# Sistemas-Multimedia/VCF

Hardware: AMD Instinct MI355X
Metric: Mpixels/s encode (DCT+deadzone) at 4K (higher is better)
Workload: dtype f32; 1 GPU; dct_dz_encode 2160x3840x3 u8 RGB frames (4K), B=8, YCoCg, deadzone Q=32, subband layout, 64 frames/step/GPU resident in HBM; global_batch=64, block_size=8, QSS=32, parallelism=frame-sharded x1

## Files before the change

vcf_amd/csrc/ab/vcf_dct_dz_ab.hip:

```cpp
#include <hip/hip_runtime.h>

#include <algorithm>
#include <cstdint>

#include "vcf_amd.h"
#include "vcf_amd_ab.h"
#include "vcf_dct8.h"
#include "vcf_dct_block.h"
#include "vcf_internal.h"
#include "vcf_pipeline.h"

namespace vcf {
namespace {

typedef uint32_t u32x4 __attribute__((ext_vector_type(4)));
typedef uint32_t u32x2 __attribute__((ext_vector_type(2)));

constexpr int kTile = 256;
constexpr int kSegBytes = kTile * 3;
constexpr int kStageBytes = 64 * kSegBytes;

struct Geom {
    int H, W, Hp, Wp, top, left, nbx, nby, tiles_per_row;
    int nblocks, tiles_per_frame;
// ... 80 lines not shown
    constexpr int per_lane = nseg * cps / kTile;
    static_assert(nseg * cps % kTile == 0, "whole stores per lane");
    const int tid = threadIdx.x;
    u32x4 v[per_lane];
    uint32_t go[per_lane];
    bool edge[per_lane];
    const uint32_t segA = (uint32_t)g.nby * (uint32_t)g.Wp * 3u, segB = (uint32_t)g.nbx * 3u;
    if (FA && SUB && segA < (1u << 24)) {
        static_assert(!SUB || (cps == 48 && bpb == 3), "multiply-shift constants");
#pragma unroll
        for (int r = 0; r < per_lane; ++r) {
            const int q = tid + r * kTile;
            const int seg = (int)(__umul24((uint32_t)q, 21846u) >> 20);
            const int off = (q - seg * cps) << 4;
            const int blk = (int)(__umul24((uint32_t)off, 43691u) >> 17);
            go[r] = rowbase[blk] + __umul24((uint32_t)(seg >> 3), segA) + __umul24((uint32_t)(seg & 7), segB) +
                    (uint32_t)(off - blk * bpb);
            v[r] = *reinterpret_cast<const u32x4 *>(stage + seg * lds_stride + off);
            edge[r] = off < 128 || off + 16 > cps * 16 - 128;
        }
    } else {
#pragma unroll
        for (int r = 0; r < per_lane; ++r) {
            const int q = tid + r * kTile;
            const int seg = q / cps;
            const int off = (q - seg * cps) << 4;
            const int blk = off / bpb;
            go[r] = rowbase[blk] + seg_base<SUB>(g, seg) + (uint32_t)(off - blk * bpb);
            v[r] = *reinterpret_cast<const u32x4 *>(stage + seg * lds_stride + off);
            edge[r] = off < 128 || off + 16 > cps * 16 - 128;
        }
    }
#pragma unroll
    for (int r = 0; r < per_lane; ++r) {
        if (NT == 1 || (NT == 2 && !edge[r]))
            __builtin_nontemporal_store(v[r] ^ 0x80808080u, reinterpret_cast<u32x4 *>(frame + go[r]));
        else
            *reinterpret_cast<u32x4 *>(frame + go[r]) = v[r] ^ 0x80808080u;
    }
}

__device__ __forceinline__ void opaque(uint32_t (&raw)[8][6], uint32_t dep)
{
#pragma unroll
    for (int y = 0; y < 8; ++y)
#pragma unroll
        for (int w = 0; w < 6; ++w) asm volatile("" : "+v"(raw[y][w]) : "v"(dep));
}

template <bool PAD, int LD = 1, bool FA = false>
__device__ __forceinline__ void load_block(const Geom &g, const uint8_t *src, int by, int bx,
                                           uint32_t (&raw)[8][6])
{
    if (!PAD) {
        const uint8_t *blk = src + ((long long)by * 8 * g.W + bx * 8) * 3;
#pragma unroll
        for (int y = 0; y < 8; ++y) {
            const u32x2 *p = reinterpret_cast<const u32x2 *>(
                FA ? blk + (long long)y * (3LL * g.W) : src + ((long long)(by * 8 + y) * g.W + bx * 8) * 3);
            const u32x2 a = LD == 0 ? __builtin_nontemporal_load(p) : p[0];
            const u32x2 b = LD == 0 ? __builtin_nontemporal_load(p + 1) : p[1];
            const u32x2 c = LD == 0 ? __builtin_nontemporal_load(p + 2) : p[2];
            raw[y][0] = a.x; raw[y][1] = a.y; raw[y][2] = b.x;
            raw[y][3] = b.y; raw[y][4] = c.x; raw[y][5] = c.y;
        }
    } else {
#pragma unroll
        for (int y = 0; y < 8; ++y) {
            const int sy = by * 8 + y - g.top;
#pragma unroll
            for (int w = 0; w < 6; ++w) raw[y][w] = 0;
#pragma unroll
            for (int n = 0; n < 24; ++n) {
                const int sx = bx * 8 + n / 3 - g.left;
                uint32_t b = 0;
                if (sy >= 0 && sy < g.H && sx >= 0 && sx < g.W)
                    b = src[((long long)sy * g.W + sx) * 3 + n % 3];
                raw[y][n >> 2] |= b << ((n & 3) * 8);
            }
        }
    }
}

template <bool POW2, bool SUB, bool PERC, bool SDWA, bool PK = false, bool MEMONLY = false>
__device__ __forceinline__ void encode_block(uint32_t (&raw)[8][6], const EncConsts &K, const FinalK &rowk,
                                             uint8_t *stage, int tid)
{
    auto s0 = [&](int i, int j, uint32_t w) {
        if (SUB) stage[(i * 8 + j) * kSegBytes + tid * 3 + 0] = (uint8_t)w;
        else stage[i * (kTile * 24) + tid * 24 + j * 3 + 0] = (uint8_t)w;
    };
    auto s1 = [&](int i, int j, uint32_t w) {
        if (SUB) stage[(i * 8 + j) * kSegBytes + tid * 3 + 1] = (uint8_t)w;
        else stage[i * (kTile * 24) + tid * 24 + j * 3 + 1] = (uint8_t)w;
    };
    auto s2 = [&](int i, int j, uint32_t w) {
        if (SUB) stage[(i * 8 + j) * kSegBytes + tid * 3 + 2] = (uint8_t)w;
        else stage[i * (kTile * 24) + tid * 24 + j * 3 + 2] = (uint8_t)w;
    };
    if constexpr (MEMONLY) {
#pragma unroll
        for (int n = 0; n < 64; ++n) {
            const uint32_t w = raw[n >> 3][(n * 3 / 4) % 6] >> (8 * (n & 3));
            s0(n >> 3, n & 7, w);
            s1(n >> 3, n & 7, w >> 1);
            s2(n >> 3, n & 7, w >> 2);
        }
    } else if constexpr (PK && POW2 && !PERC) {
        encode_block_channel_pk<0>(raw, rowk, K.qd[0], s0);
        opaque(raw, (uint32_t)tid);
        encode_block_channel_pk<1>(raw, rowk, K.qd[0], s1);
        opaque(raw, (uint32_t)tid);
        encode_block_channel_pk<2>(raw, rowk, K.qd[0], s2);
    } else {
        encode_block_channel_fold<0, POW2, PERC, SDWA>(raw, rowk, K.qd, s0);
        opaque(raw, (uint32_t)tid);
        encode_block_channel_fold<1, POW2, PERC, SDWA>(raw, rowk, K.qd, s1);
        opaque(raw, (uint32_t)tid);
        encode_block_channel_fold<2, POW2, PERC, SDWA>(raw, rowk, K.qd, s2);
    }
}

template <bool POW2, bool SUB, bool PERC, bool PAD, bool SDWA = true, bool PK = false, bool MEMONLY = false,
          int STREAMS = 0, int NT = 0, bool XCD = true, int LD = 1, int PRIO = 15, bool FA = true>
__global__ __launch_bounds__(kTile) void dct_dz_encode_kernel(const uint8_t *__restrict__ rgb,
                                                              uint8_t *__restrict__ kout, Geom g,
                                                              EncConsts K, FinalK rowk)
{
    __shared__ __attribute__((aligned(16))) uint8_t stage[kStageBytes];
    __shared__ uint32_t rowbase[kTile];
    const int tid = threadIdx.x;
    long long frame = blockIdx.y;
    int tile = blockIdx.x;
    if (XCD) {
        const unsigned n = gridDim.x * gridDim.y, gid = blockIdx.y * gridDim.x + blockIdx.x;
        const unsigned q = n >> 3, r = n & 7, x = gid & 7;
        const unsigned t = x * q + min(x, r) + (gid >> 3);
        frame = t / gridDim.x;
        tile = (int)(t - (unsigned)frame * gridDim.x);
    }
    const int n0 = tile * kTile;
    const int nvalid = min(kTile, g.nblocks - n0);
    if (tid < nvalid) {
        int by, bx;
        tile_block(g, n0 + tid, by, bx);
        rowbase[tid] = block_rowbase<SUB>(g, by, bx);
        uint32_t raw[8][6];
        if (PRIO & 3) __builtin_amdgcn_s_setprio(PRIO & 3);
        load_block<PAD, LD, FA>(g, rgb + frame * g.in_stride, by, bx, raw);
        if (PRIO & 3) __builtin_amdgcn_s_setprio(0);
        encode_block<POW2, SUB, PERC, SDWA, PK, MEMONLY>(raw, K, rowk, stage, tid);
    }
    __syncthreads();
    if (PRIO >> 2) __builtin_amdgcn_s_setprio(PRIO >> 2);
    if (STREAMS) {
        const long long S = (long long)g.out_stride * gridDim.y / 64 / 4096 * 4096;
        const long long t = (long long)blockIdx.y * gridDim.x + blockIdx.x;
        const int shift = STREAMS == 2 ? 32 : 0;
        if (nvalid == kTile)
#pragma unroll
            for (int r = 0; r < 12; ++r) {
                const int q = tid + r * kTile, seg = q / 48, off = (q - seg * 48) * 16;
                if (t * 768 + shift + off + 16 <= S)
                    __builtin_nontemporal_store(*reinterpret_cast<const u32x4 *>(stage + q * 16),
                                                reinterpret_cast<u32x4 *>(kout + seg * S + t * 768 + shift + off));
            }
        return;
    }
    if (nvalid == kTile && g.vec) move_runs_full<SUB, NT, FA>(g, stage, rowbase, kout + frame * g.out_stride);
    else move_runs_tab<SUB, true>(g, stage, rowbase, kout + frame * g.out_stride, nvalid);
}

template <bool PK>
__global__ __launch_bounds__(kTile, 2) void dct_dz_encode_diag(uint8_t *__restrict__ kout, Geom g,
                                                               EncConsts K, FinalK rowk, long long nblocks)
{
    const long long gid = (long long)blockIdx.x * kTile + threadIdx.x;
    if (gid >= nblocks) return;
    uint32_t raw[8][6];
#pragma unroll
    for (int y = 0; y < 8; ++y)
#pragma unroll
        for (int w = 0; w < 6; ++w) raw[y][w] = (uint32_t)(gid * 2654435761u) ^ (y * 0x01010101u * (w + 1));
    uint32_t acc = 0;
    auto sink = [&](int i, int j, uint32_t w) { acc += w << ((i + j) & 7); };
    if constexpr (PK) {
        encode_block_channel_pk<0>(raw, rowk, K.qd[0], sink);
        opaque(raw, acc);
        encode_block_channel_pk<1>(raw, rowk, K.qd[0], sink);
        opaque(raw, acc);
        encode_block_channel_pk<2>(raw, rowk, K.qd[0], sink);
    } else {
        encode_block_channel_fold<0, true, false, true>(raw, rowk, K.qd, sink);
        opaque(raw, acc);
        encode_block_channel_fold<1, true, false, true>(raw, rowk, K.qd, sink);
        opaque(raw, acc);
        encode_block_channel_fold<2, true, false, true>(raw, rowk, K.qd, sink);
    }
    reinterpret_cast<uint32_t *>(kout)[gid] = acc;
}

__device__ __forceinline__ void wave_lds_fence()
{
    __builtin_amdgcn_fence(__ATOMIC_SEQ_CST, "wavefront");
    __builtin_amdgcn_wave_barrier();
}

template <int TB>
struct ColsSmem {
    float tr[TB][8][9];
    uint8_t stage[64 * TB * 3 + 8 * 32];
};

template <int TB, bool SUB>
__device__ __forceinline__ int cols_stage_off(int seg)
{
    return SUB ? seg * (TB * 3) + (seg >> 3) * 32 : seg * (TB * 24) + seg * 32;
}

template <int TB, bool POW2, bool SUB, bool PERC, bool PAD>
__global__ __launch_bounds__(TB * 8) void dct_dz_encode_cols(const uint8_t *__restrict__ rgb,
                                                              uint8_t *__restrict__ kout, Geom g,
                                                              EncConsts K, int tiles_per_row)
{
    __shared__ __attribute__((aligned(16))) ColsSmem<TB> sm;
    const int tid = threadIdx.x;
    const int lb = tid >> 3, x = tid & 7;
    const int by = blockIdx.x / tiles_per_row;
    const int bx0 = (blockIdx.x - by * tiles_per_row) * TB;
    const int nvalid = min(TB, g.nbx - bx0);
    const int bx = bx0 + lb;
    const uint8_t *src = rgb + blockIdx.y * g.in_stride;
    uint8_t *dst = kout + blockIdx.y * g.out_stride;
    if (lb < nvalid) {
// ... 445 lines not shown
}

void make_geom(int32_t H, int32_t W, Geom &g)
{
    g.H = H;
    g.W = W;
    g.Hp = (H + 7) / 8 * 8;
    g.Wp = (W + 7) / 8 * 8;
    g.top = (g.Hp - H) / 2;
    g.left = (g.Wp - W) / 2;
    g.nbx = g.Wp / 8;
    g.nby = g.Hp / 8;
    g.tiles_per_row = (g.nbx + kTile - 1) / kTile;
    g.nblocks = g.nbx * g.nby;
    g.tiles_per_frame = (g.nblocks + kTile - 1) / kTile;
    g.in_stride = (long long)H * W * 3;
    g.out_stride = (long long)g.Hp * g.Wp * 3;
    g.vec = (g.nbx % 16 == 0) ? 1 : 0;
}

int check_args(const void *a, const void *b, int64_t n_frames, int32_t H, int32_t W,
               int32_t block_size, int32_t Q, uint32_t flags, bool decode)
{
    if (!a || !b) return set_error(VCF_ERR_INVALID, "null buffer");
    if (n_frames < 0) return set_error(VCF_ERR_INVALID, "n_frames < 0");
    if (H <= 0 || W <= 0)
        return set_error(VCF_ERR_INVALID, "Input image must be a 3D array (height, width, channels).");
    if (block_size != 8)
        return set_error(VCF_ERR_INVALID, "block_size %d: the 8x8 kernels need B=8", block_size);
    if (Q < 1 || (decode && Q > 32767))
        return set_error(VCF_ERR_INVALID, "quantization step %d out of range", Q);
    if (!decode && (Q & (Q - 1)) != 0 && Q > (1 << 18))
        return set_error(VCF_ERR_UNSUPPORTED, "quantization step %d too large", Q);
    if (flags & ~(VCF_DCT_NO_SUBBANDS | VCF_DCT_PERCEPTUAL))
        return set_error(VCF_ERR_INVALID, "unknown flags 0x%x", flags);
    if ((long long)((H + 7) & ~7) * ((W + 7) & ~7) * 3 >= (1LL << 31))
        return set_error(VCF_ERR_INVALID, "frame too large");
    return VCF_OK;
}

}
}

using namespace vcf;

#define VCF_ENC_CASE(P2, SB, PC, PD)                                                      \
    if (pow2 == P2 && sub == SB && perc == PC && pad == PD)                               \
        hipLaunchKernelGGL((dct_dz_encode_kernel<P2, SB, PC, PD>), grid, dim3(kTile), 0,  \
                           (hipStream_t)stream, rgb_dev + f0 * g.in_stride,               \
                           k_dev + f0 * g.out_stride, g, K, rowk);

#define VCF_DEC_CASE(SB, PC, PD)                                                          \
    if (sub == SB && perc == PC && pad == PD)                                             \
        hipLaunchKernelGGL((dct_dz_decode_kernel<SB, PC, PD>), grid, dim3(kTile), 0,      \
                           (hipStream_t)stream, k_dev + f0 * g.out_stride,                \
                           rgb_dev + f0 * g.in_stride, g, (int)Q);

extern "C" {

int vcf_dct_padded_shape(int32_t H, int32_t W, int32_t block_size, int32_t *Hp, int32_t *Wp)
{
    if (!Hp || !Wp) return set_error(VCF_ERR_INVALID, "null pointer");
    if (H <= 0 || W <= 0 || block_size <= 0)
        return set_error(VCF_ERR_INVALID, "bad shape %d x %d / block %d", H, W, block_size);
    *Hp = (H + block_size - 1) / block_size * block_size;
    *Wp = (W + block_size - 1) / block_size * block_size;
    return VCF_OK;
}

int vcf_dct_dz_encode(const uint8_t *rgb_dev, int64_t n_frames, int32_t H, int32_t W,
                      int32_t block_size, int32_t Q, uint32_t flags, uint8_t *k_dev, void *stream)
{
    return vcf_dct_dz_encode_variant(0, rgb_dev, n_frames, H, W, block_size, Q, flags, k_dev, stream);
}

int vcf_dct_dz_encode_variant(int variant, const uint8_t *rgb_dev, int64_t n_frames, int32_t H,
                              int32_t W, int32_t block_size, int32_t Q, uint32_t flags,
                              uint8_t *k_dev, void *stream)
{
    if (block_size != 8 && variant == 0)
        return dct_any_encode_u8(rgb_dev, n_frames, H, W, block_size, Q, flags, k_dev, stream);
    int rc = check_args(rgb_dev, k_dev, n_frames, H, W, block_size, Q, flags, false);
    if (rc != VCF_OK) return rc;
    if (variant < 0 || variant > 19) return set_error(VCF_ERR_INVALID, "unknown encode variant %d", variant);
    if (n_frames == 0) return VCF_OK;
    Geom g;
    make_geom(H, W, g);
    if (variant == 18 || variant == 19) {
        const PipeShape ps{2, variant == 18 ? 2 : 4, false};
        return run_pipelined(n_frames, ps, (hipStream_t)stream,
                             [&](long long f0, long long n, hipStream_t cs, const PipeHook *) {
                                 return vcf_dct_dz_encode_variant(0, rgb_dev + f0 * g.in_stride, n, H, W, block_size,
                                                                  Q, flags, k_dev + f0 * g.out_stride, cs);
                             });
    }
    const bool pow2 = (Q & (Q - 1)) == 0;
    const bool sub = !(flags & VCF_DCT_NO_SUBBANDS);
    const bool perc = (flags & VCF_DCT_PERCEPTUAL) != 0;
    const bool pad = (g.Hp != H) || (g.Wp != W);
    EncConsts K;
    make_enc_consts(K, Q);
    const FinalK rowk = pow2 ? row_final_k(Q) : final_k(1.0f, 1.0f);
    if (variant == 2 || variant == 6) {
        if (!pow2) return set_error(VCF_ERR_INVALID, "diagnostic variant needs a power-of-two Q");
        const long long nblocks = (long long)n_frames * g.nbx * g.nby;
        if (variant == 6)
            hipLaunchKernelGGL(dct_dz_encode_diag<true>, dim3((unsigned)((nblocks + kTile - 1) / kTile)),
                               dim3(kTile), 0, (hipStream_t)stream, k_dev, g, K, rowk, nblocks);
        else
            hipLaunchKernelGGL(dct_dz_encode_diag<false>, dim3((unsigned)((nblocks + kTile - 1) / kTile)),
                               dim3(kTile), 0, (hipStream_t)stream, k_dev, g, K, rowk, nblocks);
        return hip_check(hipGetLastError(), "dct_dz_encode_diag launch");
    }
    if (variant == 4) {
        if (!(pow2 && sub && !perc && !pad)) return set_error(VCF_ERR_INVALID, "variant 4: pow2 Q, aligned, default flags");
        for (int64_t f0 = 0; f0 < n_frames; f0 += 65535) {
            const dim3 grid(g.tiles_per_frame, (unsigned)std::min<int64_t>(65535, n_frames - f0));
            hipLaunchKernelGGL((dct_dz_encode_kernel<true, true, false, false, false>), grid, dim3(kTile), 0,
                               (hipStream_t)stream, rgb_dev + f0 * g.in_stride, k_dev + f0 * g.out_stride, g, K, rowk);
        }
        return hip_check(hipGetLastError(), "variant 4 launch");
    }
    if (variant == 8 || variant == 9 || variant == 10) {
        if (!(sub && !pad)) return set_error(VCF_ERR_INVALID, "variant 8: aligned frames, subband layout");
        if (variant != 8 && n_frames > 65535) return set_error(VCF_ERR_INVALID, "variants 9/10: <= 65535 frames");
        for (int64_t f0 = 0; f0 < n_frames; f0 += 65535) {
            const dim3 grid(g.tiles_per_frame, (unsigned)std::min<int64_t>(65535, n_frames - f0));
            if (variant == 8)
                hipLaunchKernelGGL((dct_dz_encode_kernel<true, true, false, false, true, false, true>), grid,
                                   dim3(kTile), 0, (hipStream_t)stream, rgb_dev + f0 * g.in_stride,
                                   k_dev + f0 * g.out_stride, g, K, rowk);
            else if (variant == 9)
                hipLaunchKernelGGL((dct_dz_encode_kernel<true, true, false, false, true, false, true, 1>), grid,
                                   dim3(kTile), 0, (hipStream_t)stream, rgb_dev, k_dev, g, K, rowk);
            else
                hipLaunchKernelGGL((dct_dz_encode_kernel<true, true, false, false, true, false, true, 2>), grid,
                                   dim3(kTile), 0, (hipStream_t)stream, rgb_dev, k_dev, g, K, rowk);
        }
        return hip_check(hipGetLastError(), "variant 8 launch");
    }
    if (variant >= 12 && variant <= 16) {
        if (!(pow2 && !perc && sub && !pad)) return set_error(VCF_ERR_INVALID, "variants 12-16: pow2 Q, aligned, default flags");
        if (n_frames > 65535) return set_error(VCF_ERR_INVALID, "variants 12-16: <= 65535 frames");
        const dim3 grid(g.tiles_per_frame, (unsigned)n_frames);
#define VCF_ENC_PRIO(V, P) \
        if (variant == V) \
            hipLaunchKernelGGL((dct_dz_encode_kernel<true, true, false, false, true, true, false, 0, 0, true, 1, P>), grid, \
                               dim3(kTile), 0, (hipStream_t)stream, rgb_dev, k_dev, g, K, rowk);
        VCF_ENC_PRIO(12, 15) VCF_ENC_PRIO(13, 5) VCF_ENC_PRIO(14, 12) VCF_ENC_PRIO(15, 3) VCF_ENC_PRIO(16, 0)
#undef VCF_ENC_PRIO
        return hip_check(hipGetLastError(), "variant 12-16 launch");
    }
    if (variant == 17) {
        if (!(pow2 && !perc && sub && !pad)) return set_error(VCF_ERR_INVALID, "variant 17: pow2 Q, aligned, default flags");
        if (n_frames > 65535) return set_error(VCF_ERR_INVALID, "variant 17: <= 65535 frames");
        const dim3 grid(g.tiles_per_frame, (unsigned)n_frames);
        hipLaunchKernelGGL((dct_dz_encode_kernel<true, true, false, false, true, true, false, 0, 0, true, 1, 15, false>),
                           grid, dim3(kTile), 0, (hipStream_t)stream, rgb_dev, k_dev, g, K, rowk);
        return hip_check(hipGetLastError(), "variant 17 launch");
    }
    if (variant == 11) {
        if (!(pow2 && !perc && sub && !pad)) return set_error(VCF_ERR_INVALID, "variant 11: pow2 Q, aligned, default flags");
        if (n_frames > 65535) return set_error(VCF_ERR_INVALID, "variant 11: <= 65535 frames");
        const dim3 grid(g.tiles_per_frame, (unsigned)n_frames);
        hipLaunchKernelGGL((dct_dz_encode_kernel<true, true, false, false, true, true, false, 0, 0, true, 0>), grid,
                           dim3(kTile), 0, (hipStream_t)stream, rgb_dev, k_dev, g, K, rowk);
        return hip_check(hipGetLastError(), "variant 11 launch");
    }
    if (variant == 7 && pow2 && !perc && sub && !pad) {
        if (n_frames > 65535) return set_error(VCF_ERR_INVALID, "variant 7: <= 65535 frames");
        const dim3 grid(g.tiles_per_frame, (unsigned)n_frames);
        hipLaunchKernelGGL((dct_dz_encode_kernel<true, true, false, false, true, true, false, 0, 1, false>), grid,
                           dim3(kTile), 0, (hipStream_t)stream, rgb_dev, k_dev, g, K, rowk);
        return hip_check(hipGetLastError(), "variant 7 launch");
    }
    if ((variant == 5 || (variant == 0 && pow2 && !perc)) && pow2 && !perc) {
        for (int64_t f0 = 0; f0 < n_frames; f0 += 65535) {
            const dim3 grid(g.tiles_per_frame, (unsigned)std::min<int64_t>(65535, n_frames - f0));
#define VCF_ENC_PK(SB, PD)                                                                                  \
    if (sub == SB && pad == PD)                                                                             \
        hipLaunchKernelGGL((dct_dz_encode_kernel<true, SB, false, PD, true, true>), grid, dim3(kTile), 0,   \
                           (hipStream_t)stream, rgb_dev + f0 * g.in_stride, k_dev + f0 * g.out_stride, g, K, rowk);
            VCF_ENC_PK(true, false) else VCF_ENC_PK(true, true) else VCF_ENC_PK(false, false) else VCF_ENC_PK(false, true)
#undef VCF_ENC_PK
            rc = hip_check(hipGetLastError(), "dct_dz_encode_kernel (packed) launch");
            if (rc != VCF_OK) return rc;
        }
        return VCF_OK;
    }
    if (variant == 3) return launch_cols<128>(rgb_dev, n_frames, k_dev, g, K, pow2, sub, perc, pad, stream);
    for (int64_t f0 = 0; f0 < n_frames; f0 += 65535) {
        const dim3 grid(g.tiles_per_frame, (unsigned)std::min<int64_t>(65535, n_frames - f0));
        VCF_ENC_CASE(true, true, false, false) else VCF_ENC_CASE(true, true, false, true)
        else VCF_ENC_CASE(true, true, true, false) else VCF_ENC_CASE(true, true, true, true)
        else VCF_ENC_CASE(true, false, false, false) else VCF_ENC_CASE(true, false, false, true)
        else VCF_ENC_CASE(true, false, true, false) else VCF_ENC_CASE(true, false, true, true)
        else VCF_ENC_CASE(false, true, false, false) else VCF_ENC_CASE(false, true, false, true)
        else VCF_ENC_CASE(false, true, true, false) else VCF_ENC_CASE(false, true, true, true)
        else VCF_ENC_CASE(false, false, false, false) else VCF_ENC_CASE(false, false, false, true)
        else VCF_ENC_CASE(false, false, true, false) else VCF_ENC_CASE(false, false, true, true)
        rc = hip_check(hipGetLastError(), "dct_dz_encode_kernel launch");
        if (rc != VCF_OK) return rc;
    }
    return VCF_OK;
}

int vcf_dct_dz_decode(const uint8_t *k_dev, int64_t n_frames, int32_t H, int32_t W,
                      int32_t block_size, int32_t Q, uint32_t flags, uint8_t *rgb_dev, void *stream)
{
    return vcf_dct_dz_decode_variant(0, k_dev, n_frames, H, W, block_size, Q, flags, rgb_dev, stream);
}

int vcf_dct_dz_decode_variant(int variant, const uint8_t *k_dev, int64_t n_frames, int32_t H, int32_t W,
                              int32_t block_size, int32_t Q, uint32_t flags, uint8_t *rgb_dev, void *stream)
{
    if (block_size != 8 && variant == 0)
        return dct_any_decode_u8(k_dev, n_frames, H, W, block_size, Q, flags, rgb_dev, stream);
    int rc = check_args(k_dev, rgb_dev, n_frames, H, W, block_size, Q, flags, true);
    if (rc != VCF_OK) return rc;
    if (variant < 0 || variant > 13) return set_error(VCF_ERR_INVALID, "unknown decode variant %d", variant);
    if (n_frames == 0) return VCF_OK;
    Geom g;
    make_geom(H, W, g);
    const bool sub = !(flags & VCF_DCT_NO_SUBBANDS);
    const bool perc = (flags & VCF_DCT_PERCEPTUAL) != 0;
    const bool pad = (g.Hp != H) || (g.Wp != W);
    if (variant >= 3) {
        if (!(sub && !perc && !pad)) return set_error(VCF_ERR_INVALID, "decode variants 3/4: aligned, default flags");
        if (n_frames > 65535) return set_error(VCF_ERR_INVALID, "decode variants 3/4: <= 65535 frames");
        const int tpr = (g.nbx + 31) / 32;
        const dim3 grid(tpr * g.nby, (unsigned)n_frames);
        if (variant == 3)
            hipLaunchKernelGGL((dct_dz_decode_cols<32, true, false, false, true, true>), grid, dim3(256), 0,
                               (hipStream_t)stream, k_dev, rgb_dev, g, (int)Q, tpr);
        else if (variant == 4)
            hipLaunchKernelGGL((dct_dz_decode_cols<32, true, false, false, false, false>), grid, dim3(256), 0,
                               (hipStream_t)stream, k_dev, rgb_dev, g, (int)Q, tpr);
        else if (variant == 5)
            hipLaunchKernelGGL((dct_dz_decode_cols<32, true, false, false, false, true, 0>), grid, dim3(256), 0,
                               (hipStream_t)stream, k_dev, rgb_dev, g, (int)Q, tpr);
        else if (variant == 6)
            hipLaunchKernelGGL((dct_dz_decode_cols<32, true, false, false, false, true, 3, 1>), grid, dim3(256), 0,
// ... 40 lines not shown
```

vcf_amd/csrc/vcf_dct_block.h:

```cpp
#pragma once
#include <math.h>
#include <stdint.h>
#include <string.h>

#include "vcf_dct8.h"

#if defined(__HIP_DEVICE_COMPILE__)
#define VCF_OPAQUE(x) asm volatile("" : "+v"(x))
#define VCF_SCHED_FENCE() __builtin_amdgcn_sched_barrier(0)
#else
#define VCF_OPAQUE(x) ((void)0)
#define VCF_SCHED_FENCE() ((void)0)
#endif

#if defined(__HIPCC__)
#define VCF_HD_HOST __host__
#else
#define VCF_HD_HOST
#endif

namespace vcf {

constexpr unsigned char kYQ[64] = {
    16, 11, 10, 16, 24, 40, 51, 61,   12, 12, 14, 19, 26, 58, 60, 55,
// ... 449 lines not shown
template <int B1>
VCF_HD uint32_t twice_byte(uint32_t b)
{
#if defined(__HIP_DEVICE_COMPILE__) && VCF_SDWA_ASM
    constexpr int B0 = -1;
    const uint32_t a = 1;
    VCF_SDWA_FN("v_lshlrev_b32_sdwa")
#else
    return byte_sel<B1>(b) << 1;
#endif
}

template <int C, int X>
VCF_HD float ycocg_sdwa(const uint32_t (&row)[6], uint32_t magic)
{
    constexpr int nr = 3 * X, ng = 3 * X + 1, nb = 3 * X + 2;
    const uint32_t wr = row[nr >> 2], wg = row[ng >> 2], wb = row[nb >> 2];
    if (C == 0) {
        const uint32_t rb = add_sdwa<nr & 3, nb & 3>(wr, wb);
        return bits_as_float(rb + twice_byte<ng & 3>(wg) + magic) - (8388608.0f + 512.0f);
    }
    if (C == 1) {
        const uint32_t t = add_sdwa<-1, nr & 3>(magic, wr);
        return bits_as_float(sub_sdwa<-1, nb & 3>(t, wb)) - (8388608.0f + 256.0f);
    }
    const uint32_t rb = add_sdwa<nr & 3, nb & 3>(wr, wb);
    const uint32_t t = add_sdwa<-1, ng & 3>(magic - rb, wg);
    return bits_as_float(add_sdwa<-1, ng & 3>(t, wg)) - (8388608.0f + 512.0f);
}

template <int C>
VCF_HD constexpr uint32_t ycocg_magic_word()
{
    return C == 0 ? kMagicI : C == 1 ? kMagicI + 256u : kMagicI + 512u;
}

template <int C, int X, bool SDWA>
VCF_HD void fold_columns(const uint32_t (&raw)[8][6], uint32_t magic, const FinalK &colk, float (&v)[8][8],
                         float &dep)
{
    if constexpr (X < 8) {
        float col[8];
#pragma unroll
        for (int y = 0; y < 8; ++y)
            col[y] = SDWA ? ycocg_sdwa<C, X>(raw[y], magic)
                          : ycocg_magic<C>(byte_of(raw[y], 3 * X), byte_of(raw[y], 3 * X + 1),
                                           byte_of(raw[y], 3 * X + 2));
        chain8(col, dep);
        dct2_8f(col, colk);
#pragma unroll
        for (int y = 0; y < 8; ++y) v[y][X] = col[y];
        dep = col[0];
        fold_columns<C, X + 1, SDWA>(raw, magic, colk, v, dep);
    }
}

template <int C, bool POW2, bool PERC, bool SDWA = false, typename Sink>
VCF_HD void encode_block_channel_fold(const uint32_t (&raw)[8][6], const FinalK &rowk, const float (&qd)[4],
                                      Sink &&sink)
{
    constexpr float cs = C == 1 ? 0.5f : 0.25f;
    constexpr FinalK colk = POW2 ? final_k(cs * 0.25f, cs * 0.5f) : final_k(1.0f, 1.0f);
    float v[8][8];
    float dep = qd[0];
    uint32_t magic = ycocg_magic_word<C>();
    VCF_OPAQUE(magic);
    fold_columns<C, 0, SDWA>(raw, magic, colk, v, dep);
#pragma unroll
    for (int i = 0; i < 8; ++i) {
        chain8(v[i], dep);
        if (POW2) dct2_8f(v[i], rowk);
        else dct2_8r(v[i]);
        dep = v[i][0];
#pragma unroll
        for (int j = 0; j < 8; ++j) {
            float t = v[i][j];
            if (PERC) t = (float)((double)t * pweight<C>(i * 8 + j));
            const float q = POW2 ? t : quant_div<false>(t, qd[qexp<C>(i, j) - 3]);
            sink(i, j, (uint32_t)cvt_trunc_i32(q));
        }
    }
}

#if defined(__HIPCC__)
typedef float vcf_f2 __attribute__((ext_vector_type(2)));
typedef uint32_t vcf_u2 __attribute__((ext_vector_type(2)));

template <int C, int X>
VCF_HD uint32_t ycocg_bits_sdwa(const uint32_t (&row)[6], uint32_t magic)
{
    constexpr int nr = 3 * X, ng = 3 * X + 1, nb = 3 * X + 2;
    const uint32_t wr = row[nr >> 2], wg = row[ng >> 2], wb = row[nb >> 2];
    if (C == 0) return add_sdwa<nr & 3, nb & 3>(wr, wb) + twice_byte<ng & 3>(wg) + magic;
    if (C == 1) return sub_sdwa<-1, nb & 3>(add_sdwa<-1, nr & 3>(magic, wr), wb);
    const uint32_t rb = add_sdwa<nr & 3, nb & 3>(wr, wb);
    return add_sdwa<-1, ng & 3>(add_sdwa<-1, ng & 3>(magic - rb, wg), wg);
}

template <int C, int XP>
VCF_HD void fold_columns_pk(const uint32_t (&raw)[8][6], uint32_t magic, const FinalK &colk,
                            vcf_f2 (&v)[8][4], vcf_f2 &dep)
{
    if constexpr (XP < 4) {
        constexpr float centre = C == 1 ? 8388608.0f + 256.0f : 8388608.0f + 512.0f;
        vcf_f2 col[8];
#pragma unroll
        for (int y = 0; y < 8; ++y) {
            const vcf_u2 b = {ycocg_bits_sdwa<C, 2 * XP>(raw[y], magic),
                              ycocg_bits_sdwa<C, 2 * XP + 1>(raw[y], magic)};
            col[y] = __builtin_bit_cast(vcf_f2, b) - centre;
        }
        chain8(col, dep);
        dct2_8f(col, colk);
#pragma unroll
        for (int y = 0; y < 8; ++y) v[y][XP] = col[y];
        dep = col[0];
        fold_columns_pk<C, XP + 1>(raw, magic, colk, v, dep);
    }
}

template <int C, typename Sink>
VCF_HD void encode_block_channel_pk(const uint32_t (&raw)[8][6], const FinalK &rowk, float dep0, Sink &&sink)
{
    constexpr float cs = C == 1 ? 0.5f : 0.25f;
    constexpr FinalK colk = final_k(cs * 0.25f, cs * 0.5f);
    vcf_f2 v[8][4];
    vcf_f2 dep = {dep0, dep0};
    uint32_t magic = ycocg_magic_word<C>();
    VCF_OPAQUE(magic);
    fold_columns_pk<C, 0>(raw, magic, colk, v, dep);
#pragma unroll
    for (int p = 0; p < 4; ++p) {
        vcf_f2 r[8];
#pragma unroll
        for (int xp = 0; xp < 4; ++xp) {
            r[2 * xp] = __builtin_shufflevector(v[2 * p][xp], v[2 * p + 1][xp], 0, 2);
            r[2 * xp + 1] = __builtin_shufflevector(v[2 * p][xp], v[2 * p + 1][xp], 1, 3);
        }
        chain8(r, dep);
        dct2_8f(r, rowk);
        dep = r[0];
#pragma unroll
        for (int j = 0; j < 8; ++j) {
            sink(2 * p, j, (uint32_t)cvt_trunc_i32(r[j].x));
            sink(2 * p + 1, j, (uint32_t)cvt_trunc_i32(r[j].y));
        }
    }
}
#endif

VCF_HD uint32_t byte_at(const uint32_t (&K)[16], int n)
{
    return (K[n >> 2] >> (8 * (n & 3))) & 0xffu;
}

template <int C, bool PERC>
VCF_HD void decode_block_channel(const uint8_t (&kb)[64], int Q, uint32_t (&res)[32])
{
    double v[8][8];
#pragma unroll
    for (int n = 0; n < 64; ++n) {
        int16_t y = (int16_t)(Q * ((int)kb[n] - 128));
        if (PERC) {
            const float f = (float)((double)(float)y / pweight<C>(n));
            y = (int16_t)(int)f;
        }
        v[n >> 3][n & 7] = (double)y;
    }
#pragma unroll
    for (int x = 0; x < 8; ++x) {
        double col[8];
#pragma unroll
        for (int y = 0; y < 8; ++y) col[y] = v[y][x];
        dct3_8r(col);
#pragma unroll
        for (int y = 0; y < 8; ++y) v[y][x] = col[y];
    }
#pragma unroll
    for (int y = 0; y < 8; ++y) dct3_8r(v[y]);
#pragma unroll
    for (int n = 0; n < 32; ++n) {
        const uint32_t lo = (uint16_t)(int16_t)(int)(v[(2 * n) >> 3][(2 * n) & 7] * 0.0625);
        const uint32_t hi = (uint16_t)(int16_t)(int)(v[(2 * n + 1) >> 3][(2 * n + 1) & 7] * 0.0625);
        res[n] = lo | (hi << 16);
    }
#pragma unroll
    for (int n = 0; n < 32; ++n) VCF_OPAQUE(res[n]);
}

VCF_HD uint32_t clip_u8(int v)
{
    v = (int16_t)(v + 128);
    return (uint32_t)(v < 0 ? 0 : (v > 255 ? 255 : v));
}

VCF_HD int sample_of(const uint32_t (&p)[32], int n)
{
    return (int16_t)(uint16_t)(p[n >> 1] >> ((n & 1) * 16));
}

VCF_HD void to_rgb_row(const uint32_t (&Yv)[32], const uint32_t (&Co)[32], const uint32_t (&Cg)[32],
                       int y, uint32_t (&px)[24])
{
#pragma unroll
    for (int x = 0; x < 8; ++x) {
        const int n = y * 8 + x;
        const int yv = sample_of(Yv, n), co = sample_of(Co, n), cg = sample_of(Cg, n);
        px[3 * x + 0] = clip_u8((int16_t)(yv + co - cg));
        px[3 * x + 1] = clip_u8((int16_t)(yv + cg));
        px[3 * x + 2] = clip_u8((int16_t)(yv - co - cg));
    }
#pragma unroll
    for (int q = 0; q < 24; ++q) VCF_OPAQUE(px[q]);
}

// ... 2 lines not shown
```

vcf_amd/csrc/vcf_dct_dz.hip:

```cpp
#include <hip/hip_runtime.h>

#include <algorithm>
#include <cstdint>

#include "vcf_amd.h"
#include "vcf_dct8.h"
#include "vcf_dct_block.h"
#include "vcf_internal.h"

namespace vcf {
namespace {

typedef uint32_t u32x4 __attribute__((ext_vector_type(4)));
typedef uint32_t u32x2 __attribute__((ext_vector_type(2)));

constexpr int kTile = 256;

struct Geom {
    int H, W, Hp, Wp, top, left, nbx, nby, tiles_per_row;
    int nblocks, tiles_per_frame;
    long long in_stride, out_stride;
    int vec;
};

// ... 87 lines not shown
    if (SUB && segA < (1u << 24)) {
        static_assert(!SUB || bpb == 3, "multiply-shift constants");
#pragma unroll
        for (int r = 0; r < per_lane; ++r) {
            const int q = tid + r * T;
            const int seg = (int)(__umul24((uint32_t)q, DivCps<T>::m) >> DivCps<T>::s);
            const int off = (q - seg * cps) << 4;
            const int blk = (int)(__umul24((uint32_t)off, 683u) >> 11);
            go[r] = rowbase[blk] + __umul24((uint32_t)(seg >> 3), segA) + __umul24((uint32_t)(seg & 7), segB) +
                    (uint32_t)(off - blk * bpb);
            v[r] = *reinterpret_cast<const u32x4 *>(stage + seg * lds_stride + off);
        }
    } else {
#pragma unroll
        for (int r = 0; r < per_lane; ++r) {
            const int q = tid + r * T;
            const int seg = q / cps;
            const int off = (q - seg * cps) << 4;
            const int blk = off / bpb;
            go[r] = rowbase[blk] + seg_base<SUB>(g, seg) + (uint32_t)(off - blk * bpb);
            v[r] = *reinterpret_cast<const u32x4 *>(stage + seg * lds_stride + off);
        }
    }
#pragma unroll
    for (int r = 0; r < per_lane; ++r) *reinterpret_cast<u32x4 *>(frame + go[r]) = v[r] ^ 0x80808080u;
}

__device__ __forceinline__ void opaque(uint32_t (&raw)[8][6], uint32_t dep)
{
#pragma unroll
    for (int y = 0; y < 8; ++y)
#pragma unroll
        for (int w = 0; w < 6; ++w) asm volatile("" : "+v"(raw[y][w]) : "v"(dep));
}

template <bool PAD>
__device__ __forceinline__ void load_block(const Geom &g, const uint8_t *src, int by, int bx,
                                           uint32_t (&raw)[8][6])
{
    if (!PAD) {
        const uint8_t *blk = src + ((long long)by * 8 * g.W + bx * 8) * 3;
#pragma unroll
        for (int y = 0; y < 8; ++y) {
            const u32x2 *p = reinterpret_cast<const u32x2 *>(blk + (long long)y * (3LL * g.W));
            const u32x2 a = p[0], b = p[1], c = p[2];
            raw[y][0] = a.x; raw[y][1] = a.y; raw[y][2] = b.x;
            raw[y][3] = b.y; raw[y][4] = c.x; raw[y][5] = c.y;
        }
    } else {
#pragma unroll
        for (int y = 0; y < 8; ++y) {
            const int sy = by * 8 + y - g.top;
#pragma unroll
            for (int w = 0; w < 6; ++w) raw[y][w] = 0;
#pragma unroll
            for (int n = 0; n < 24; ++n) {
                const int sx = bx * 8 + n / 3 - g.left;
                uint32_t b = 0;
                if (sy >= 0 && sy < g.H && sx >= 0 && sx < g.W)
                    b = src[((long long)sy * g.W + sx) * 3 + n % 3];
                raw[y][n >> 2] |= b << ((n & 3) * 8);
            }
        }
    }
}

template <bool POW2, bool SUB, bool PERC, bool PK, int T = kTile>
__device__ __forceinline__ void encode_block(uint32_t (&raw)[8][6], const EncConsts &K, const FinalK &rowk,
                                             uint8_t *stage, int tid)
{
    auto s0 = [&](int i, int j, uint32_t w) {
        if (SUB) stage[(i * 8 + j) * (T * 3) + tid * 3 + 0] = (uint8_t)w;
        else stage[i * (T * 24) + tid * 24 + j * 3 + 0] = (uint8_t)w;
    };
    auto s1 = [&](int i, int j, uint32_t w) {
        if (SUB) stage[(i * 8 + j) * (T * 3) + tid * 3 + 1] = (uint8_t)w;
        else stage[i * (T * 24) + tid * 24 + j * 3 + 1] = (uint8_t)w;
    };
    auto s2 = [&](int i, int j, uint32_t w) {
        if (SUB) stage[(i * 8 + j) * (T * 3) + tid * 3 + 2] = (uint8_t)w;
        else stage[i * (T * 24) + tid * 24 + j * 3 + 2] = (uint8_t)w;
    };
    if constexpr (PK && POW2 && !PERC) {
        encode_block_channel_pk<0>(raw, rowk, K.qd[0], s0);
        opaque(raw, (uint32_t)tid);
        encode_block_channel_pk<1>(raw, rowk, K.qd[0], s1);
        opaque(raw, (uint32_t)tid);
        encode_block_channel_pk<2>(raw, rowk, K.qd[0], s2);
    } else {
        encode_block_channel_fold<0, POW2, PERC, true>(raw, rowk, K.qd, s0);
        opaque(raw, (uint32_t)tid);
        encode_block_channel_fold<1, POW2, PERC, true>(raw, rowk, K.qd, s1);
        opaque(raw, (uint32_t)tid);
        encode_block_channel_fold<2, POW2, PERC, true>(raw, rowk, K.qd, s2);
    }
}

template <bool POW2, bool SUB, bool PERC, bool PAD, bool PK, int T = kTile>
__global__ __launch_bounds__(T) void dct_dz_encode_kernel(const uint8_t *__restrict__ rgb,
                                                          uint8_t *__restrict__ kout, Geom g,
                                                          EncConsts K, FinalK rowk)
{
    __shared__ __attribute__((aligned(16))) uint8_t stage[64 * T * 3];
    __shared__ uint32_t rowbase[T];
    const int tid = threadIdx.x;
    const unsigned n = gridDim.x * gridDim.y, gid = blockIdx.y * gridDim.x + blockIdx.x;
    const unsigned q = n >> 3, r = n & 7, xcd = gid & 7;
    const unsigned t = xcd * q + min(xcd, r) + (gid >> 3);
    const long long frame = t / gridDim.x;
    const int tile = (int)(t - (unsigned)frame * gridDim.x);
    const int n0 = tile * T;
    const int nvalid = min(T, g.nblocks - n0);
    if (tid < nvalid) {
        int by, bx;
        tile_block(g, n0 + tid, by, bx);
        rowbase[tid] = block_rowbase<SUB>(g, by, bx);
        uint32_t raw[8][6];
        __builtin_amdgcn_s_setprio(3);
        load_block<PAD>(g, rgb + frame * g.in_stride, by, bx, raw);
        __builtin_amdgcn_s_setprio(0);
        encode_block<POW2, SUB, PERC, PK, T>(raw, K, rowk, stage, tid);
    }
    __syncthreads();
    __builtin_amdgcn_s_setprio(3);
    if (nvalid == T && g.vec) move_runs_full<SUB, T>(g, stage, rowbase, kout + frame * g.out_stride);
    else move_runs_tab<SUB, true, T>(g, stage, rowbase, kout + frame * g.out_stride, nvalid);
}

__device__ __forceinline__ void wave_lds_fence()
{
    __builtin_amdgcn_fence(__ATOMIC_SEQ_CST, "wavefront");
    __builtin_amdgcn_wave_barrier();
}

template <int TB, bool SUB>
__device__ __forceinline__ int cols_stage_off(int seg)
{
    return SUB ? seg * (TB * 3) + (seg >> 3) * 32 : seg * (TB * 24) + seg * 32;
}

template <int TB>
struct DecColsSmem {
    double tr[TB][8][9];
    double lut[256];
    uint8_t stage[64 * TB * 3 + 8 * 32];
};

template <int TB, bool SUB, bool PERC, bool PAD>
__global__ __launch_bounds__(TB * 8) void dct_dz_decode_cols(const uint8_t *__restrict__ kin,
                                                              uint8_t *__restrict__ rgb, Geom g, int Q,
                                                              int tiles_per_row)
{
    constexpr bool NTL = false, NTS = true;
    constexpr int PRIO = 3, DQ = 1, EPI = 1;
    __shared__ __attribute__((aligned(16))) DecColsSmem<TB> sm;
    const int tid = threadIdx.x;
    const int lb = tid >> 3, x = tid & 7;
    const int by = blockIdx.x / tiles_per_row;
    const int bx0 = (blockIdx.x - by * tiles_per_row) * TB;
    const int nvalid = min(TB, g.nbx - bx0);
    const int bx = bx0 + lb;
    const uint8_t *src = kin + blockIdx.y * g.out_stride;
    uint8_t *dst = rgb + blockIdx.y * g.in_stride;

    constexpr int nseg = SUB ? 64 : 8;
    auto seg_off = [&](int seg) -> uint32_t {
        return (uint32_t)(SUB ? seg_offset_sub(g, by, bx0, seg) : seg_offset_nosub(g, by, bx0, seg));
    };
    if (PRIO) __builtin_amdgcn_s_setprio(PRIO);
    const uint32_t runA = (uint32_t)g.nby * (uint32_t)g.Wp * 3u, runB = (uint32_t)g.nbx * 3u;
    const bool fast24 = EPI == 1 && SUB && runA < (1u << 24) && runB * 8u < (1u << 24);
    const uint32_t runBase = ((uint32_t)by * (uint32_t)g.Wp + (uint32_t)bx0) * 3u;
    if (g.vec && nvalid == TB && (TB * 3) % 16 == 0) {
        constexpr int cps = (SUB ? 3 * TB : 24 * TB) / 16, total = nseg * cps;
        constexpr uint32_t kDivM = ((1u << 18) + cps - 1) / cps;
        static_assert(total < 4096, "multiply-shift division range");
#pragma unroll
        for (int q0 = 0; q0 < total; q0 += TB * 8) {
            const int q = q0 + tid;
            if (total % (TB * 8) == 0 || q < total) {
                int seg, off;
                uint32_t so;
                if (fast24) {
                    seg = (int)(__umul24((uint32_t)q, kDivM) >> 18);
                    off = (q - seg * cps) << 4;
                    so = __umul24((uint32_t)(seg >> 3), runA) + __umul24((uint32_t)(seg & 7), runB) + runBase;
                } else {
                    seg = q / cps;
                    off = (q - seg * cps) << 4;
                    so = seg_off(seg);
                }
                const u32x4 *gp = reinterpret_cast<const u32x4 *>(src + so + off);
                *reinterpret_cast<u32x4 *>(sm.stage + cols_stage_off<TB, SUB>(seg) + off) =
                    NTL ? __builtin_nontemporal_load(gp) : *gp;
            }
        }
    } else {
        const int seg_len = SUB ? 3 * nvalid : 24 * nvalid, total = nseg * seg_len;
#pragma clang loop unroll(disable) vectorize(disable) interleave(disable)
        for (int q = tid; q < total; q += TB * 8) {
            const int seg = q / seg_len, off = q - seg * seg_len;
            sm.stage[cols_stage_off<TB, SUB>(seg) + off] = src[seg_off(seg) + off];
        }
    }
    if (PRIO) __builtin_amdgcn_s_setprio(0);
// ... 280 lines not shown
```

Measured before the change: 723,700 Mpixels/s.

## Skip row DCT for row pairs that quantize to zero across the wave

Before each row-pair DCT pass in the packed encode path, the code sums the absolute column-pass outputs. If a ballot shows every lane's pair falls below the deadzone threshold, the row transform and quantization are skipped. In the production kernel (SKIP=2) the zero bytes are no longer written per skipped row; the staging rows 2..7 are pre-cleared with vectorized LDS stores, so skipped rows read as zero and computed rows overwrite them. The cost is the extra abs-sum and ballot per row pair plus the bulk zero fill, which pays off only when high-frequency rows are zero across whole waves. Correctness rests on the conservative bound constant.

Result: faster. 873,700 Mpixels/s, median of 6 (+20.7%).

```diff
diff --git a/vcf_amd/csrc/ab/vcf_dct_dz_ab.hip b/vcf_amd/csrc/ab/vcf_dct_dz_ab.hip
--- a/vcf_amd/csrc/ab/vcf_dct_dz_ab.hip
+++ b/vcf_amd/csrc/ab/vcf_dct_dz_ab.hip
@@ -186,7 +186,7 @@
     }
 }
 
-template <bool POW2, bool SUB, bool PERC, bool SDWA, bool PK = false, bool MEMONLY = false>
+template <bool POW2, bool SUB, bool PERC, bool SDWA, bool PK = false, bool MEMONLY = false, int SKIP = 0>
 __device__ __forceinline__ void encode_block(uint32_t (&raw)[8][6], const EncConsts &K, const FinalK &rowk,
                                              uint8_t *stage, int tid)
 {
@@ -211,11 +211,11 @@
             s2(n >> 3, n & 7, w >> 2);
         }
     } else if constexpr (PK && POW2 && !PERC) {
-        encode_block_channel_pk<0>(raw, rowk, K.qd[0], s0);
+        encode_block_channel_pk<0, SKIP>(raw, rowk, K.qd[0], s0);
         opaque(raw, (uint32_t)tid);
-        encode_block_channel_pk<1>(raw, rowk, K.qd[0], s1);
+        encode_block_channel_pk<1, SKIP>(raw, rowk, K.qd[0], s1);
         opaque(raw, (uint32_t)tid);
-        encode_block_channel_pk<2>(raw, rowk, K.qd[0], s2);
+        encode_block_channel_pk<2, SKIP>(raw, rowk, K.qd[0], s2);
     } else {
         encode_block_channel_fold<0, POW2, PERC, SDWA>(raw, rowk, K.qd, s0);
         opaque(raw, (uint32_t)tid);
@@ -226,7 +226,7 @@
 }
 
 template <bool POW2, bool SUB, bool PERC, bool PAD, bool SDWA = true, bool PK = false, bool MEMONLY = false,
-          int STREAMS = 0, int NT = 0, bool XCD = true, int LD = 1, int PRIO = 15, bool FA = true>
+          int STREAMS = 0, int NT = 0, bool XCD = true, int LD = 1, int PRIO = 15, bool FA = true, int SKIP = 0>
 __global__ __launch_bounds__(kTile) void dct_dz_encode_kernel(const uint8_t *__restrict__ rgb,
                                                               uint8_t *__restrict__ kout, Geom g,
                                                               EncConsts K, FinalK rowk)
@@ -253,7 +253,7 @@
         if (PRIO & 3) __builtin_amdgcn_s_setprio(PRIO & 3);
         load_block<PAD, LD, FA>(g, rgb + frame * g.in_stride, by, bx, raw);
         if (PRIO & 3) __builtin_amdgcn_s_setprio(0);
-        encode_block<POW2, SUB, PERC, SDWA, PK, MEMONLY>(raw, K, rowk, stage, tid);
+        encode_block<POW2, SUB, PERC, SDWA, PK, MEMONLY, SKIP>(raw, K, rowk, stage, tid);
     }
     __syncthreads();
     if (PRIO >> 2) __builtin_amdgcn_s_setprio(PRIO >> 2);
@@ -865,7 +865,7 @@
         return dct_any_encode_u8(rgb_dev, n_frames, H, W, block_size, Q, flags, k_dev, stream);
     int rc = check_args(rgb_dev, k_dev, n_frames, H, W, block_size, Q, flags, false);
     if (rc != VCF_OK) return rc;
-    if (variant < 0 || variant > 19) return set_error(VCF_ERR_INVALID, "unknown encode variant %d", variant);
+    if (variant < 0 || variant > 21) return set_error(VCF_ERR_INVALID, "unknown encode variant %d", variant);
     if (n_frames == 0) return VCF_OK;
     Geom g;
     make_geom(H, W, g);
@@ -941,6 +941,24 @@
         hipLaunchKernelGGL((dct_dz_encode_kernel<true, true, false, false, true, true, false, 0, 0, true, 1, 15, false>),
                            grid, dim3(kTile), 0, (hipStream_t)stream, rgb_dev, k_dev, g, K, rowk);
         return hip_check(hipGetLastError(), "variant 17 launch");
+    }
+    if (variant == 20 || variant == 21) {
+        if (!(pow2 && !perc)) return set_error(VCF_ERR_INVALID, "variants 20/21: pow2 Q, no -p");
+        for (int64_t f0 = 0; f0 < n_frames; f0 += 65535) {
+            const dim3 grid(g.tiles_per_frame, (unsigned)std::min<int64_t>(65535, n_frames - f0));
+#define VCF_ENC_SKIP(SB, PD, SK)                                                                                   \
+    if (sub == SB && pad == PD && (variant == 21) == (SK == 1))                                                     \
+        hipLaunchKernelGGL((dct_dz_encode_kernel<true, SB, false, PD, true, true, false, 0, 0, true, 1, 15, true, SK>), \
+                           grid, dim3(kTile), 0, (hipStream_t)stream, rgb_dev + f0 * g.in_stride,                   \
+                           k_dev + f0 * g.out_stride, g, K, rowk);
+            VCF_ENC_SKIP(true, false, 0) else VCF_ENC_SKIP(true, true, 0) else VCF_ENC_SKIP(false, false, 0)
+            else VCF_ENC_SKIP(false, true, 0) else VCF_ENC_SKIP(true, false, 1) else VCF_ENC_SKIP(true, true, 1)
+            else VCF_ENC_SKIP(false, false, 1) else VCF_ENC_SKIP(false, true, 1)
+#undef VCF_ENC_SKIP
+            rc = hip_check(hipGetLastError(), "variant 20/21 launch");
+            if (rc != VCF_OK) return rc;
+        }
+        return VCF_OK;
     }
     if (variant == 11) {
         if (!(pow2 && !perc && sub && !pad)) return set_error(VCF_ERR_INVALID, "variant 11: pow2 Q, aligned, default flags");
diff --git a/vcf_amd/csrc/vcf_dct_block.h b/vcf_amd/csrc/vcf_dct_block.h
--- a/vcf_amd/csrc/vcf_dct_block.h
+++ b/vcf_amd/csrc/vcf_dct_block.h
@@ -555,6 +555,50 @@
     }
 }
 
+constexpr float kRowSkipC = 4.0f + 0.00390625f;
+
+VCF_HD float row_skip_scale(float qd0)
+{
+    return qd0 * kRowSkipC;
+}
+
+VCF_HD float abs_f(float x)
+{
+#if defined(__HIPCC__)
+    return __builtin_fabsf(x);
+#else
+    return fabsf(x);
+#endif
+}
+
+VCF_HD float abs_add(float a, float b)
+{
+    float s = abs_f(a) + abs_f(b);
+#if defined(__HIP_DEVICE_COMPILE__)
+    asm("" : "+v"(s));
+#endif
+    return s;
+}
+
+VCF_HD float row_abs_sum(float a0, float a1, float a2, float a3, float a4, float a5, float a6, float a7)
+{
+    return abs_add(abs_add(abs_add(a0, a1), abs_add(a2, a3)), abs_add(abs_add(a4, a5), abs_add(a6, a7)));
+}
+
+VCF_HD bool row_pair_is_zero(float sa, float sb, float kb)
+{
+    return __builtin_fmaxf(sa, sb) * kb < 1.0f;
+}
+
+VCF_HD bool wave_all(bool pred)
+{
+#if defined(__HIP_DEVICE_COMPILE__)
+    return __builtin_amdgcn_ballot_w64(!pred) == 0;
+#else
+    return pred;
+#endif
+}
+
 #if defined(__HIPCC__)
 typedef float vcf_f2 __attribute__((ext_vector_type(2)));
 typedef uint32_t vcf_u2 __attribute__((ext_vector_type(2)));
@@ -592,7 +636,7 @@
     }
 }
 
-template <int C, typename Sink>
+template <int C, int SKIP = 0, typename Sink>
 VCF_HD void encode_block_channel_pk(const uint32_t (&raw)[8][6], const FinalK &rowk, float dep0, Sink &&sink)
 {
     constexpr float cs = C == 1 ? 0.5f : 0.25f;
@@ -602,8 +646,24 @@
     uint32_t magic = ycocg_magic_word<C>();
     VCF_OPAQUE(magic);
     fold_columns_pk<C, 0>(raw, magic, colk, v, dep);
+    const float kb = row_skip_scale(dep0);
 #pragma unroll
     for (int p = 0; p < 4; ++p) {
+        if (SKIP && p > 0) {
+            const vcf_f2(&a)[4] = v[2 * p], (&b)[4] = v[2 * p + 1];
+            const float sa = row_abs_sum(a[0].x, a[0].y, a[1].x, a[1].y, a[2].x, a[2].y, a[3].x, a[3].y);
+            const float sb = row_abs_sum(b[0].x, b[0].y, b[1].x, b[1].y, b[2].x, b[2].y, b[3].x, b[3].y);
+            if (wave_all(row_pair_is_zero(sa, sb, kb))) {
+                if (SKIP == 1) {
+#pragma unroll
+                    for (int j = 0; j < 8; ++j) {
+                        sink(2 * p, j, 0u);
+                        sink(2 * p + 1, j, 0u);
+                    }
+                }
+                continue;
+            }
+        }
         vcf_f2 r[8];
 #pragma unroll
         for (int xp = 0; xp < 4; ++xp) {
diff --git a/vcf_amd/csrc/vcf_dct_dz.hip b/vcf_amd/csrc/vcf_dct_dz.hip
--- a/vcf_amd/csrc/vcf_dct_dz.hip
+++ b/vcf_amd/csrc/vcf_dct_dz.hip
@@ -193,11 +193,11 @@
         else stage[i * (T * 24) + tid * 24 + j * 3 + 2] = (uint8_t)w;
     };
     if constexpr (PK && POW2 && !PERC) {
-        encode_block_channel_pk<0>(raw, rowk, K.qd[0], s0);
+        encode_block_channel_pk<0, 2>(raw, rowk, K.qd[0], s0);
         opaque(raw, (uint32_t)tid);
-        encode_block_channel_pk<1>(raw, rowk, K.qd[0], s1);
+        encode_block_channel_pk<1, 2>(raw, rowk, K.qd[0], s1);
         opaque(raw, (uint32_t)tid);
-        encode_block_channel_pk<2>(raw, rowk, K.qd[0], s2);
+        encode_block_channel_pk<2, 2>(raw, rowk, K.qd[0], s2);
     } else {
         encode_block_channel_fold<0, POW2, PERC, true>(raw, rowk, K.qd, s0);
         opaque(raw, (uint32_t)tid);
@@ -205,6 +205,29 @@
         opaque(raw, (uint32_t)tid);
         encode_block_channel_fold<2, POW2, PERC, true>(raw, rowk, K.qd, s2);
     }
+}
+
+template <bool SUB, int T>
+__device__ __forceinline__ void zero_wave_rows(uint8_t *stage, int tid)
+{
+    const int w = tid >> 6, l = tid & 63;
+    const u32x4 z = {0u, 0u, 0u, 0u};
+    if (SUB) {
+        if ((l & 15) < 12) {
+            uint8_t *p = stage + (16 + (l >> 4)) * (T * 3) + w * 192 + (l & 15) * 16;
+#pragma unroll
+            for (int r = 0; r < 12; ++r) *reinterpret_cast<u32x4 *>(p + r * 4 * (T * 3)) = z;
+        }
+    } else {
+        uint8_t *p = stage + 2 * (T * 24) + w * 1536 + l * 16;
+#pragma unroll
+        for (int i = 0; i < 6; ++i) {
+            *reinterpret_cast<u32x4 *>(p + i * (T * 24)) = z;
+            if (l < 32) *reinterpret_cast<u32x4 *>(p + i * (T * 24) + 1024) = z;
+        }
+    }
+    __builtin_amdgcn_fence(__ATOMIC_RELEASE, "wavefront");
+    __builtin_amdgcn_wave_barrier();
 }
 
 template <bool POW2, bool SUB, bool PERC, bool PAD, bool PK, int T = kTile>
@@ -222,16 +245,17 @@
     const int tile = (int)(t - (unsigned)frame * gridDim.x);
     const int n0 = tile * T;
     const int nvalid = min(T, g.nblocks - n0);
+    uint32_t raw[8][6];
     if (tid < nvalid) {
         int by, bx;
         tile_block(g, n0 + tid, by, bx);
         rowbase[tid] = block_rowbase<SUB>(g, by, bx);
-        uint32_t raw[8][6];
         __builtin_amdgcn_s_setprio(3);
         load_block<PAD>(g, rgb + frame * g.in_stride, by, bx, raw);
         __builtin_amdgcn_s_setprio(0);
-        encode_block<POW2, SUB, PERC, PK, T>(raw, K, rowk, stage, tid);
-    }
+    }
+    if constexpr (PK && POW2 && !PERC) zero_wave_rows<SUB, T>(stage, tid);
+    if (tid < nvalid) encode_block<POW2, SUB, PERC, PK, T>(raw, K, rowk, stage, tid);
     __syncthreads();
     __builtin_amdgcn_s_setprio(3);
     if (nvalid == T && g.vec) move_runs_full<SUB, T>(g, stage, rowbase, kout + frame * g.out_stride);
```
